# GT-STAR-Lab/MARBLER

Hardware: AMD Instinct MI355X
Metric: env agent-steps/sec (higher is better)
Workload: dtype f32

## Files before the change

marbler_amd/csrc/step_group.h:

```cpp
#pragma once
#include <hip/hip_runtime.h>
#include <stdint.h>

#include <type_traits>

#include "device_common.h"
#include "ipm_qp.h"
#include "lidar.h"
#include "team.h"
#include "probes/diag.h"

namespace rg {

__device__ __forceinline__ void out_store4(float *p, float a, float b, float c, float d) {
    *reinterpret_cast<float4 *>(p) = make_float4(a, b, c, d);
}
__device__ __forceinline__ void out_store1(float *p, float a) {
    *p = a;
}

constexpr int CHUNK = RG_CHUNK;
static_assert(CHUNK >= 1 && CHUNK <= 5, "the sparse collision pre-test covers sub-steps 0..2 and 3..4 of a chunk: longer chunks would go untested");

template <int GW, int QPM = 0, typename QpLds = void, bool SPAN = false>
__device__ __forceinline__ int controller(const rg_scenario_params &p, const Consts &k, int N, int ag, bool lane_ok,
                                          bool upd, float x, float y, float c, float s, float gx, float gy, float &v,
                                          float &w, QpLds *qp RG_CTRL_TICKS_PARAM) {
    RG_CTRL_BEGIN(x, y, c, s)
    const float xix = x + k.pd * c, xiy = y + k.pd * s;
    float ux = gx - xix, uy = gy - xiy;
    {
        const float nrm = norm2_spec(ux, uy);
        const float sc = k.pvl / nrm;
        const bool clip = nrm > k.pvl;
        ux = clip ? ux * sc : ux;
        uy = clip ? uy * sc : uy;
    }
    if constexpr (QPM == RG_QP_CVXOPT) {
        {
            const float n2u = ux * ux + uy * uy;
            const bool clip = n2u > k.bml * k.bml;
            if (__any(clip)) {
                const float sc = k.bml / __builtin_sqrtf(n2u);
                ux = clip ? ux * sc : ux;
                uy = clip ? uy * sc : uy;
            }
        }
        const int lane_ = threadIdx.x;
        qp->rec[lane_] = make_float4(xix, xiy, ux, uy);
        __syncthreads();
        int iters = 0;
        if (upd) iters = ipm::solve_qp_n<GW>(N, ipm::make_consts(p), qp->rec + (lane_ & ~(GW - 1)), qp->ws[lane_ / GW], ag);
        __syncthreads();
        const float4 r = qp->rec[lane_];
        ux = r.z;
        uy = r.w;
        RG_CTRL_TICK(1);
        float vv = c * ux + s * uy;
        float ww = k.inv_pd * (-s * ux + c * uy);
        ww = ww > k.wlim ? k.wlim : ww;
        ww = ww < -k.wlim ? -k.wlim : ww;
        vv = vv > k.vmax ? k.vmax : vv;
        vv = vv < -k.vmax ? -k.vmax : vv;
        ww = ww > k.wmax ? k.wmax : ww;
        ww = ww < -k.wmax ? -k.wmax : ww;
        v = upd ? vv : v;
        w = upd ? ww : w;
        RG_CTRL_TICK(2);
        return iters;
    }
    const float bgain = p.barrier_gain, ugain = p.unsafe_barrier_gain, qp_rtol = p.qp_rtol;
    const int qp_cap = p.qp_max_sweeps;
    const bool has_unsafe = p.barrier_has_unsafe_gain != 0;
    float ex[GW - 1], ey[GW - 1], fx[GW - 1], fy[GW - 1], bp[GW - 1], emax[GW - 1];
    float mu[GW - 1], dmu[GW - 1];
    auto pair_consts = [&](float pxi, float pyi, int K, int i) {
        const float dx = xix - pxi, dy = xiy - pyi;
        const float ee = dx * dx + dy * dy;
        const float h = ee - k.r2;
        const float gain = ((h >= 0.0f) | !has_unsafe) ? bgain : ugain;
        const float b = gain * ((h * h) * h);
        const float n2 = 2.0f * ee;
        const bool ok = lane_ok & ((ag ^ K) < N) & (n2 > 0.0f);
        const float rn2 = ok ? 1.0f / n2 : 0.0f;
        ex[i] = dx;
        ey[i] = dy;
        fx[i] = dx * rn2;
        fy[i] = dy * rn2;
        bp[i] = (0.5f * b) * rn2;
        emax[i] = ok ? fmaxf(__builtin_fabsf(dx), __builtin_fabsf(dy)) : 0.0f;
    };
    const bool helper = SPAN && (threadIdx.x & GW) != 0;
    if constexpr (SPAN) {
        static_assert(GW == 8, "16-lane rows of two 8-lane halves");
        const float mx = mirror_upper_half(xix), my = mirror_upper_half(xiy);
        static_for<0, 4>([&](auto SS) {
            constexpr int S = decltype(SS)::value;
            const int K = helper ? S ^ 7 : S;
            if constexpr (S == 0) pair_consts(mx, my, K, 6);
            else pair_consts(xor_lane<S>(mx), xor_lane<S>(my), K, (S ^ 7) - 1);
        });
        static_for<1, 4>([&](auto SS) {
            constexpr int S = decltype(SS)::value, J = (S ^ 7) - 1;
            ex[S - 1] = ex[J];
            ey[S - 1] = ey[J];
            fx[S - 1] = fx[J];
            fy[S - 1] = fy[J];
            bp[S - 1] = bp[J];
            emax[S - 1] = emax[J];
        });
        static_for<3, 7>([&](auto JJ) {
            constexpr int J = decltype(JJ)::value;
            ex[J] = to_lower_half(ex[J]);
            ey[J] = to_lower_half(ey[J]);
            fx[J] = to_lower_half(fx[J]);
            fy[J] = to_lower_half(fy[J]);
            bp[J] = to_lower_half(bp[J]);
            emax[J] = to_lower_half(emax[J]);
        });
    } else {
        static_for<1, GW>([&](auto KK) {
            constexpr int K = decltype(KK)::value;
            pair_consts(xor_lane<K>(xix), xor_lane<K>(xiy), K, K - 1);
        });
    }
    static_for<0, GW - 1>([&](auto KK) { mu[decltype(KK)::value] = dmu[decltype(KK)::value] = 0.0f; });
    RG_CTRL_PIN_ROUNDS(GW, fx, bp, emax)
    RG_CTRL_TICK(0);
    {
        const float n2u = ux * ux + uy * uy;
        const bool clip = n2u > k.bml * k.bml;
        if (__any(clip)) {
            const float sc = k.bml / __builtin_sqrtf(n2u);
            ux = clip ? ux * sc : ux;
            uy = clip ? uy * sc : uy;
        }
    }
    const float uhx = ux, uhy = uy;
    bool active = upd & !helper;
    int sweeps = 0, my_sweeps = 0;
    auto sweep = [&](auto PH) {
        constexpr int PHASE = decltype(PH)::value;
        ++sweeps;
        if (active) {
            float chg = 0.0f, pa = 0.0f, pb = 0.0f;
            static_for<1, GW>([&](auto KK) {
                constexpr int K = decltype(KK)::value;
                const float pux = xor_lane<K>(ux), puy = xor_lane<K>(uy);
                const float c0 = mu[K - 1] - bp[K - 1];
                const float t = __builtin_fmaf(fy[K - 1], puy - uy, c0);
                float mn = __builtin_fmaf(fx[K - 1], pux - ux, t);
                mn = (mn > 0.0f) ? mn : 0.0f;
                const float delta = mn - mu[K - 1];
                mu[K - 1] = mn;
                ux = __builtin_fmaf(delta, ex[K - 1], ux);
                uy = __builtin_fmaf(delta, ey[K - 1], uy);
                chg = fmaxf(chg, __builtin_fabsf(delta) * emax[K - 1]);
                if constexpr (PHASE == 2) dmu[K - 1] = delta;
                if constexpr (PHASE == 3) {
                    const float dd = delta - dmu[K - 1];
                    pa = __builtin_fmaf(dd, delta, pa);
                    pb = __builtin_fmaf(dd, dd, pb);
                    dmu[K - 1] = delta;
                }
            });
            my_sweeps = sweeps;
            const float um = lane_ok ? fmaxf(__builtin_fabsf(ux), __builtin_fabsf(uy)) : 0.0f;
            const float gchg = group_max_nonneg<GW>(chg);
            const float gum = fmaxf(k.bml, group_max_nonneg<GW>(um));
            active = (gchg > qp_rtol * gum) & (sweeps < qp_cap);
            if constexpr (PHASE == 3) {
                if (active) {
                    const float ga = group_sum<GW>(pa), gb = group_sum<GW>(pb);
                    const bool ok = (gb > 0.0f) & (ga < 0.0f) & (-ga < 32.0f * gb);
                    const float gam = ok ? ga / gb : 0.0f;
                    float sx = uhx, sy = uhy;
                    static_for<1, GW>([&](auto KK) {
                        constexpr int K = decltype(KK)::value;
                        float m = __builtin_fmaf(-gam, dmu[K - 1], mu[K - 1]);
                        m = (m > 0.0f) ? m : 0.0f;
                        mu[K - 1] = m;
                        sx = __builtin_fmaf(m, ex[K - 1], sx);
                        sy = __builtin_fmaf(m, ey[K - 1], sy);
                    });
                    ux = sx;
                    uy = sy;
                }
            }
        }
    };
    if constexpr (SPAN) {
        while (active) {
            sweep(std::integral_constant<int, 1>{});
            if (!active) break;
            sweep(std::integral_constant<int, 2>{});
            if (!active) break;
            sweep(std::integral_constant<int, 3>{});
            if (!active) break;
            sweep(std::integral_constant<int, 0>{});
        }
    } else {
        while (__any(active)) {
            sweep(std::integral_constant<int, 1>{});
            if (!__any(active)) break;
            sweep(std::integral_constant<int, 2>{});
            if (!__any(active)) break;
            sweep(std::integral_constant<int, 3>{});
            if (!__any(active)) break;
            sweep(std::integral_constant<int, 0>{});
        }
    }
    if constexpr (SPAN) {
        ux = to_upper_half(ux);
        uy = to_upper_half(uy);
    }
    RG_CTRL_PIN2(ux, uy);
    RG_CTRL_TICK(1);
    float vv = c * ux + s * uy;
    float ww = k.inv_pd * (-s * ux + c * uy);
    ww = ww > k.wlim ? k.wlim : ww;
    ww = ww < -k.wlim ? -k.wlim : ww;
    vv = vv > k.vmax ? k.vmax : vv;
    vv = vv < -k.vmax ? -k.vmax : vv;
    ww = ww > k.wmax ? k.wmax : ww;
    ww = ww < -k.wmax ? -k.wmax : ww;
    v = upd ? vv : v;
    w = upd ? ww : w;
    RG_CTRL_PIN2(v, w);
    RG_CTRL_COUNT_SWEEPS(sweeps);
    RG_CTRL_TICK(2);
    return my_sweeps;
}

template <int GW, int OD, int NT>
__device__ __forceinline__ void write_neighbour_obs(Lds<GW> &lds, int N, int Knb, int ag, int gbase, bool lane_ok,
                                                    float x, float y, float *obs_row) {
    constexpr int M = NT > 0 ? NT - 1 : GW - 1;
    unsigned long long key[M > 0 ? M : 1];
    bool ok[M > 0 ? M : 1];
    int rank[M > 0 ? M : 1], who[M > 0 ? M : 1];
    static_for<0, M>([&](auto RR) {
        constexpr int r = decltype(RR)::value;
        int j = ag + r + 1;
        j = j >= N ? j - N : j;
        j = j & (GW - 1);
        who[r] = j;
        const float2 pxy = *reinterpret_cast<const float2 *>(&lds.own[gbase + j][0]);
        const float dx = pxy.x - x, dy = pxy.y - y;
        const float d2 = dx * dx + dy * dy;
        ok[r] = lane_ok & (r + 1 < N);
        const unsigned int hi = ok[r] ? __builtin_bit_cast(unsigned int, d2) : 0xFFFFFFFFu;
        key[r] = (static_cast<unsigned long long>(hi) << 32) | static_cast<unsigned int>(j);
        rank[r] = M - 1 - r;
    });
    const bool all_others = Knb >= N - 1;
    static_for<1, M>([&](auto KK) {
        constexpr int k = decltype(KK)::value;
        static_for<0, k>([&](auto QQ) {
            constexpr int q = decltype(QQ)::value;
            const int q_first = key[q] < key[k] ? 1 : 0;
            rank[k] += q_first;
            rank[q] -= q_first;
        });
    });
    float row[M > 0 ? M : 1][OD];
    static_for<0, M>([&](auto RR) {
        constexpr int r = decltype(RR)::value;
        const float *src = &lds.own[gbase + who[r]][0];
        if constexpr (OD == 4) {
            const float4 v = *reinterpret_cast<const float4 *>(src);
            row[r][0] = v.x;
            row[r][1] = v.y;
            row[r][2] = v.z;
            row[r][3] = v.w;
        } else {
#pragma unroll
            for (int c = 0; c < OD; ++c) row[r][c] = src[c];
        }
    });
    static_for<0, M>([&](auto RR) {
        constexpr int r = decltype(RR)::value;
        const int j = who[r];
        const int slot = all_others ? (j < ag ? j : j - 1) : rank[r];
        if (ok[r] & (all_others | (slot < Knb))) {
            float *o = obs_row + (slot + 1) * OD;
            if constexpr (OD == 4) {
                out_store4(o, row[r][0], row[r][1], row[r][2], row[r][3]);
            } else {
#pragma unroll
                for (int c = 0; c < OD; ++c) o[c] = row[r][c];
            }
        }
    });
}

template <int SCN, int GW, bool OBS_ONLY, int NT, bool AHEAD, bool GYM, int QPM = 0, typename QpLds = void, typename Sync = WgSync,
          bool LIDAR = false, bool TEAM = false, bool SPAN = false>
__device__ __forceinline__ void step_once(const KernelArgs &a, Lds<GW> &lds, const StepView &sv, QpLds *qp_lds = nullptr,
                                          const rg_lidar_params *lid = nullptr, const rg_team_params *tm = nullptr) {
    static_assert(!SPAN || (GW == 8 && QPM == 0 && !GYM && !LIDAR && !TEAM), "the 16-lane rows: exact mode, GW = 8, no side blocks");
    constexpr int RW = SPAN ? 2 * GW : GW;
    constexpr int EPW = WAVE / RW;
    RG_STAMPS_BEGIN()
    const rg_scenario_params &p = a.p;
    const Consts &k = a.k;
    const float *q_poses = a.st.poses, *q_carry = a.st.carry_dist, *q_ret = a.st.ep_return, *q_sum = a.st.done_return_sum;
    const int32_t *q_steps = a.st.episode_steps, *q_act = sv.actions, *q_cnt = a.st.done_count, *q_stp = a.st.done_steps_sum;
    int32_t *q_el = GYM ? sv.io.elapsed : nullptr;
    const int q_tl = GYM ? sv.io.time_limit : 0;
    const int32_t *q_rc = a.st.reset_count, *q_nep = AHEAD ? a.st.next_episode : nullptr;
    const float *q_nin = AHEAD ? a.st.next_init : nullptr;
    const int q_nst = AHEAD ? a.next_stride : 0;
    const int q_E = a.E, q_epw = a.envs_per_wave, q_P = p.num_prey, q_N = p.n_agents, q_G = gridDim.x;
    asm volatile("" ::"s"(q_poses), "s"(q_carry), "s"(q_ret), "s"(q_sum), "s"(q_steps), "s"(q_act), "s"(q_cnt), "s"(q_stp),
                 "s"(q_E), "s"(q_epw), "s"(q_P), "s"(q_N), "s"(q_G), "s"(q_rc));
    if constexpr (GYM) asm volatile("" ::"s"(q_el), "s"(q_tl));
    if constexpr (AHEAD) asm volatile("" ::"s"(q_nep), "s"(q_nin), "s"(q_nst));
    const float *q_prey = a.st.prey_loc;
    const uint8_t *q_sen = a.st.prey_sensed, *q_cap = a.st.prey_captured, *q_loaded = a.st.loaded, *q_grid = a.st.grid;
    const uint8_t *q_pix = a.st.pixel_type, *q_reached = a.st.reached_goal;
    const int32_t *q_gcol = a.st.goal_col, *q_msg = a.st.messages, *q_zone = a.st.zone_load, *q_load = a.st.load;
    if constexpr (SCN == RG_SCN_PREDATOR_CAPTURE_PREY) asm volatile("" ::"s"(q_prey), "s"(q_sen), "s"(q_cap));
    else if constexpr (SCN == RG_SCN_WAREHOUSE) asm volatile("" ::"s"(q_loaded));
    else if constexpr (SCN == RG_SCN_SIMPLE) asm volatile("" ::"s"(q_prey));
    else if constexpr (SCN == RG_SCN_ARCTIC_TRANSPORT) asm volatile("" ::"s"(q_grid), "s"(q_pix), "s"(q_reached), "s"(q_gcol));
    else asm volatile("" ::"s"(q_msg), "s"(q_zone), "s"(q_load));
    int32_t *q_tidx = TEAM ? tm->team_index : nullptr;
    const float *q_tstep = TEAM ? tm->agent_step : nullptr, *q_tsr = TEAM ? tm->sensing_radius : nullptr;
    const float *q_tcr = TEAM ? tm->capture_radius : nullptr;
    const int32_t *q_ttq = TEAM ? tm->torque : nullptr;
    const int q_tC = TEAM ? tm->n_sets : 1;
    if constexpr (TEAM) {
        asm volatile("" ::"s"(q_tidx), "s"(q_tstep), "s"(q_tC));
        if constexpr (SCN == RG_SCN_PREDATOR_CAPTURE_PREY) asm volatile("" ::"s"(q_tsr), "s"(q_tcr));
        else if constexpr (SCN == RG_SCN_MATERIAL_TRANSPORT) asm volatile("" ::"s"(q_ttq));
    }

    const int N = NT > 0 ? NT : q_N;
    const int lane = threadIdx.x;
    const int ag = lane & (GW - 1);
    const int g = lane / RW;
    const int gbase = lane & ~(RW - 1);
    const bool helper = SPAN && (lane & GW) != 0;
    const int epw = q_epw > 0 ? q_epw : EPW;
    const int chunk = xcd_chunk(q_G);
    const int e = chunk * epw + g;
    const bool env_ok = (g < epw) & (e < q_E);
    const bool lane_ok = env_ok && ag < N;
    const bool env_st = env_ok & !helper, lane_st = lane_ok & !helper;
    const size_t eN = static_cast<size_t>(e) * N;

#define RG_LATE(v) asm volatile("" : "+v"(v))
    float x = 0.0f, y = 0.0f, th = 0.0f, carry = 0.0f;
    int act = 4;
    int steps_raw = 0;
    float agent_step = 0.0f, sr = 0.0f, cr = 0.0f;
    float st_ret = 0.0f, st_sum = 0.0f;
    int st_cnt = 0, st_steps = 0;
    const bool stats = (!OBS_ONLY) && q_ret != nullptr;
    int pix = 0, reached = 0;
    int team_raw = 0, tq_raw = 0;
    if constexpr (TEAM) {
        if (env_ok) team_raw = q_tidx[e];
    }
    if (lane_ok) {
        const float *X = q_poses + eN * 3;
        x = X[ag];
        y = X[N + ag];
        th = X[2 * N + ag];
        if constexpr (!OBS_ONLY) act = q_act[eN + ag];
        if constexpr (SCN == RG_SCN_ARCTIC_TRANSPORT) pix = q_pix[eN + ag];
        if constexpr (!TEAM) {
        agent_step = p.agent_step[ag];
        if constexpr (SCN == RG_SCN_PREDATOR_CAPTURE_PREY) {
            sr = p.sensing_radius[ag];
            cr = p.capture_radius[ag];
        }
        }
        if constexpr (!OBS_ONLY) carry = q_carry[eN + ag];
        if constexpr (TEAM) {
            const size_t ti = static_cast<size_t>(team_clamp(team_raw, q_tC)) * N + ag;
            agent_step = q_tstep[ti];
            if constexpr (SCN == RG_SCN_PREDATOR_CAPTURE_PREY) {
                sr = q_tsr[ti];
                cr = q_tcr[ti];
            }
            if constexpr (SCN == RG_SCN_MATERIAL_TRANSPORT) tq_raw = q_ttq[ti];
        }
    }
    int rc_raw = -1;
    const bool ahead = AHEAD && (!OBS_ONLY) && q_nst > 0 && a.auto_reset;
    int nx_tag = -2;
    float nx_pose[3] = {0.0f, 0.0f, 0.0f};
    float nx_a = 0.0f, nx_b = 0.0f;
    uint32_t nx_grid[7] = {0, 0, 0, 0, 0, 0, 0};
    auto load_next = [&](bool want) {
        if (want) {
            const float *nb = q_nin + static_cast<size_t>(e) * q_nst;
            if (ag < N) {
                nx_pose[0] = nb[ag];
                nx_pose[1] = nb[N + ag];
                nx_pose[2] = nb[2 * N + ag];
            }
            if constexpr (SCN == RG_SCN_PREDATOR_CAPTURE_PREY || SCN == RG_SCN_SIMPLE) {
                if (ag < q_P) {
                    nx_a = nb[3 * N + 2 * ag];
                    nx_b = nb[3 * N + 2 * ag + 1];
                }
            } else if constexpr (SCN == RG_SCN_MATERIAL_TRANSPORT) {
                if (ag < 2) nx_a = nb[3 * N + ag];
            } else if constexpr (SCN == RG_SCN_ARCTIC_TRANSPORT) {
                const uint32_t *gb = reinterpret_cast<const uint32_t *>(nb + 3 * N);
#pragma unroll
                for (int t = 0; t < 6; ++t) nx_grid[t] = gb[ag * 6 + t];
                nx_grid[6] = gb[24];
            }
        }
    };
    int el_raw = 0;
    if (env_ok) {
        steps_raw = q_steps[e];
        if (!OBS_ONLY && a.auto_reset) rc_raw = q_rc[e];
        if constexpr (GYM) el_raw = q_el[e];
        if (ahead) nx_tag = q_nep[e];
        if (stats && ag == 0) {
            st_ret = q_ret[e];
            st_sum = q_sum[e];
            st_cnt = q_cnt[e];
            st_steps = q_stp[e];
        }
    }
    uint32_t sen_lo = 0, sen_hi = 0, cap_lo = 0, cap_hi = 0;
    int flag_raw[4] = {0, 0, 0, 0};
    int loaded = 0;
    float goal_x = 0.0f, goal_y = 0.0f;
    uint32_t grid_pre[6] = {0, 0, 0, 0, 0, 0};
    int goal_col = 1;
    int load = 0, zone0 = 0, zone1 = 0;
    int msg[4] = {0, 0, 0, 0};
    float2 prey_r[8];
#pragma unroll
    for (int t = 0; t < 8; ++t) prey_r[t] = make_float2(0.0f, 0.0f);
    static_assert(SCN != RG_SCN_ARCTIC_TRANSPORT || GW == 4, "ArcticTransport is a 4-agent scenario");
    if constexpr (SCN == RG_SCN_PREDATOR_CAPTURE_PREY) {
        const int P = q_P;
        if (P <= 8) {
            if (env_ok) {
                const float2 *src = reinterpret_cast<const float2 *>(q_prey) + static_cast<size_t>(e) * P;
#pragma unroll
                for (int t = 0; t < 8; ++t) prey_r[t] = src[t < P ? t : P - 1];
                if (ag < P) {
                    flag_raw[0] = q_sen[static_cast<size_t>(e) * P + ag];
                    flag_raw[1] = q_cap[static_cast<size_t>(e) * P + ag];
                }
                if constexpr (GW < 8)
                    if (ag + GW < P) {
                        flag_raw[2] = q_sen[static_cast<size_t>(e) * P + ag + GW];
                        flag_raw[3] = q_cap[static_cast<size_t>(e) * P + ag + GW];
                    }
            }
        } else {
            if (env_ok) {
                for (int i = ag; i < 2 * P; i += GW) lds.prey[g][i] = q_prey[static_cast<size_t>(e) * 2 * P + i];
                for (int i = ag; i < P; i += GW) {
                    const uint32_t sb = q_sen[static_cast<size_t>(e) * P + i] != 0;
                    const uint32_t cb = q_cap[static_cast<size_t>(e) * P + i] != 0;
                    if (i < 32) {
                        sen_lo |= sb << i;
                        cap_lo |= cb << i;
                    } else {
                        sen_hi |= sb << (i - 32);
                        cap_hi |= cb << (i - 32);
                    }
                }
            }
            sen_lo = group_or<GW>(sen_lo);
            cap_lo = group_or<GW>(cap_lo);
            if (P > 32) {
                sen_hi = group_or<GW>(sen_hi);
                cap_hi = group_or<GW>(cap_hi);
            }
        }
    } else if constexpr (SCN == RG_SCN_WAREHOUSE) {
        if (lane_ok) loaded = q_loaded[eN + ag];
    } else if constexpr (SCN == RG_SCN_SIMPLE) {
        if (env_ok) {
            goal_x = q_prey[static_cast<size_t>(e) * 2];
            goal_y = q_prey[static_cast<size_t>(e) * 2 + 1];
        }
    } else if constexpr (SCN == RG_SCN_ARCTIC_TRANSPORT) {
        if (env_ok) {
            const uint32_t *gsrc = reinterpret_cast<const uint32_t *>(q_grid + static_cast<size_t>(e) * 96);
#pragma unroll
            for (int t = 0; t < 6; ++t) grid_pre[t] = gsrc[ag * 6 + t];
            goal_col = q_gcol[e];
        }
        if (lane_ok) reached = q_reached[eN + ag];
    } else {
        if (env_ok) {
#pragma unroll
            for (int i = 0; i < 4; ++i) {
                if (OBS_ONLY || i >= N) msg[i] = q_msg[4 * e + i];
                else msg[i] = q_act[eN + i];
            }
            zone0 = q_zone[2 * e];
            zone1 = q_zone[2 * e + 1];
        }
        if (lane_ok) load = q_load[eN + ag];
    }

    int viol = 0, max_sweeps = 0;
    bool replayed = false;
    float dist = 0.0f;
    if constexpr (!OBS_ONLY) {
        RG_PIN5(x, y, th, carry, act);
        RG_STAMP(0);
        float gx = x, gy = y;
        {
            const int mv = (SCN == RG_SCN_MATERIAL_TRANSPORT) ? act / 4 : act;
            float sd = agent_step;
            if constexpr (SCN == RG_SCN_ARCTIC_TRANSPORT) {
                const float nrm_s = p.arctic_normal_step, slow_s = p.arctic_slow_step, fast_s = p.arctic_fast_step;
                const float water = pix == 1 ? slow_s : pix == 2 ? fast_s : nrm_s;
                const float ice = pix == 1 ? fast_s : pix == 2 ? slow_s : nrm_s;
                sd = ag < 2 ? fast_s : ag == 3 ? water : ice;
            }
            const float cgx = clamp_spec(gx, p.left, p.right), cgy = clamp_spec(gy, p.up, p.down);
            const float lft = (gx - sd) > p.left ? (gx - sd) : p.left;
            const float rgt = (gx + sd) < p.right ? (gx + sd) : p.right;
            const float upw = (gy - sd) > p.up ? (gy - sd) : p.up;
            const float dwn = (gy + sd) < p.down ? (gy + sd) : p.down;
            gx = mv == 0 ? lft : mv == 1 ? rgt : cgx;
            gy = mv == 2 ? upw : mv == 3 ? dwn : cgy;
        }
        const int thr_pre = __builtin_bit_cast(int, k.thr_pre);
        const int ghost_q = __builtin_bit_cast(int, __builtin_amdgcn_cvt_pkrtz(1000.0f + 32.0f * ag, -1000.0f));
        float v = 0.0f, w = 0.0f, s = 0.0f, c = 1.0f;
        RG_CHUNK_LOCALS()
        RG_CTRL_LOCALS()
        float acc = carry, last = 0.0f;
        bool dead = false;
        float fin_x = 0.0f, fin_y = 0.0f;
        float bx = x, by = y, ox = 0.0f, oy = 0.0f;
        const bool penalize = p.penalize_violations != 0;
        const int U = p.update_frequency, period = p.controller_period;
        for (int it0 = 0; it0 < U; it0 += period) {
            const int n = (U - it0) < period ? (U - it0) : period;
            RG_HEADING_SINCOS(th, s, c);
            const int sw = controller<GW, QPM, QpLds, SPAN>(p, k, N, ag, lane_ok, env_ok & !dead, x, y, c, s, gx, gy, v, w, qp_lds RG_CTRL_TICKS_ARG);
            max_sweeps = sw > max_sweeps ? sw : max_sweeps;
            const float dtv = k.dt * v, dtw = k.dt * w;
            float sd, cd;
            sincos_small_spec(dtw, sd, cd);
            if (__any(__builtin_fabsf(dtw) > 0.25f)) {
                float sd2, cd2;
                sincos_spec(dtw, sd2, cd2);
                const bool big = __builtin_fabsf(dtw) > 0.25f;
                sd = big ? sd2 : sd;
                cd = big ? cd2 : cd;
            }
            if (it0 == 0) RG_STAMP(1);
            const float mrg = __builtin_fmaf((CHUNK - 1) * 1.000001f, __builtin_fabsf(dtv), PRE_SLACK);
            int n_exec = n;
            bool died_now = false;
            const float mstep = lane_ok ? __builtin_fmaf(__builtin_fabsf(k.coll_off), __builtin_fabsf(dtw), __builtin_fabsf(dtv)) * 1.00001f : 0.0f;
            const float M2 = 2.0f * group_max_nonneg<GW>(mstep);
            auto thr_span = [&](int span) {
                const float t = (k.lin_pre + PRE_SLACK) + static_cast<float>(span) * M2;
                return __builtin_bit_cast(int, (t * t) * 1.00002f);
            };
            const int thr_s1 = thr_span(1), thr_s2 = thr_span(2);
            const bool sparse_ok = (k.lin_pre + 2.0f * M2) < 0.24f;

            auto run_chunk = [&](auto CC, int j0) {
                constexpr int C = decltype(CC)::value;
                const float x0 = x, y0 = y, ox0 = ox, oy0 = oy, c0 = c, s0 = s;
                const bool live = lane_ok & !dead;
                int q[C];
                const bool bnd_any = live & ((__builtin_fabsf(x - k.xc) + mrg > k.xh) | (__builtin_fabsf(y - k.yc) + mrg > k.yh));
                static_for<0, C>([&](auto UU) {
                    constexpr int u = decltype(UU)::value;
                    const float fx = __builtin_fmaf(k.coll_off, c, x), fy = __builtin_fmaf(k.coll_off, s, y);
                    const int qr = __builtin_bit_cast(int, __builtin_amdgcn_cvt_pkrtz(fx, fy));
                    q[u] = live ? qr : ghost_q;
                    ox = __builtin_fmaf(c, dtv, ox);
                    oy = __builtin_fmaf(s, dtv, oy);
                    x = bx + ox;
                    y = by + oy;
                    const float cn = __builtin_fmaf(c, cd, -(s * sd));
                    const float sn = __builtin_fmaf(s, cd, c * sd);
                    c = cn;
                    s = sn;
                });
                auto pair_min = [&](int qv) {
                    constexpr bool QUAD_COVER = GW == 8 && NT >= 5 && NT <= 7;
                    constexpr int R = QUAD_COVER ? NT - 1 : GW - 1;
                    int d[R];
                    auto diff = [&](int partner_q) {
                        return __builtin_bit_cast(int, __builtin_bit_cast(half2v, qv) - __builtin_bit_cast(half2v, partner_q));
                    };
                    if constexpr (QUAD_COVER) {
                        static_for<1, 4>([&](auto KK) { d[decltype(KK)::value - 1] = diff(xor_lane_i<decltype(KK)::value>(qv)); });
                        static_for<0, NT - 4>([&](auto MM) { d[3 + decltype(MM)::value] = diff(cross_lane_i<decltype(MM)::value>(qv)); });
                    } else {
                        static_for<1, GW>([&](auto KK) { d[decltype(KK)::value - 1] = diff(xor_lane_i<decltype(KK)::value>(qv)); });
                    }
                    int dm = 0x7FFFFFFF;
                    dot2_batch<R>(d);
#pragma unroll
                    for (int r = 0; r < R; ++r) dm = d[r] < dm ? d[r] : dm;
                    return dm;
                };
                int dmin_u[C];
                bool sparse_hit = live & !sparse_ok;
                {
                    constexpr int SPAN0 = C - 1 < 2 ? C - 1 : 2;
                    const int t0 = SPAN0 == 0 ? thr_pre : SPAN0 == 1 ? thr_s1 : thr_s2;
                    if constexpr (SPAN && C >= 4) {
                        const int t3 = C == 4 ? thr_pre : thr_s1;
                        const int dm = pair_min(helper ? q[3] : q[0]);
                        sparse_hit = sparse_hit | (dm <= (helper ? t3 : t0));
                        dmin_u[0] = dmin_u[3] = dm;
                    } else {
                        dmin_u[0] = pair_min(q[0]);
                        sparse_hit = sparse_hit | (dmin_u[0] <= t0);
                        if constexpr (C >= 4) {
                            const int t3 = C == 4 ? thr_pre : thr_s1;
                            dmin_u[3] = pair_min(q[3]);
                            sparse_hit = sparse_hit | (dmin_u[3] <= t3);
                        }
                    }
                }
                if (penalize && __any(sparse_hit | bnd_any)) {
                RG_CHUNK_DENSE_BEGIN()
                if constexpr (SPAN && C >= 4) {
                    const int mine = dmin_u[0], other = xor_lane_i<8>(mine);
                    dmin_u[0] = helper ? other : mine;
                    dmin_u[3] = helper ? mine : other;
                }
                if constexpr (SPAN && C >= 3) {
                    const int mine = pair_min(helper ? q[2] : q[1]), other = xor_lane_i<8>(mine);
                    if constexpr (C == 5) dmin_u[4] = pair_min(q[4]);
                    dmin_u[1] = helper ? other : mine;
                    dmin_u[2] = helper ? mine : other;
                } else {
                    static_for<1, C>([&](auto UU) {
                        constexpr int u = decltype(UU)::value;
                        if constexpr (u != 3) dmin_u[u] = pair_min(q[u]);
                    });
                }
                int dmin = dmin_u[0];
                static_for<1, C>([&](auto UU) { dmin = dmin_u[decltype(UU)::value] < dmin ? dmin_u[decltype(UU)::value] : dmin; });
                RG_CHUNK_DENSE_END(dmin)
                if (__any((dmin <= thr_pre) | bnd_any)) {
                    replayed = true;
                    float rx = x0, ry = y0, rox = ox0, roy = oy0, rc = c0, rs = s0;
                    static_for<0, C>([&](auto UU) {
                        constexpr int u = decltype(UU)::value;
                        const bool bnd = lane_ok & !dead & ((rx < k.xmin) | (rx > k.xmax) | (ry < k.ymin) | (ry > k.ymax));
                        const float fx = __builtin_fmaf(k.coll_off, rc, rx), fy = __builtin_fmaf(k.coll_off, rs, ry);
                        bool col = false;
                        if (!__any(dmin_u[u] <= thr_pre)) {
                        } else if constexpr (GW == 8 && NT >= 5 && NT <= 7) {
                            static_for<1, 4>([&](auto KK) {
                                constexpr int K = decltype(KK)::value;
                                const float dx = fx - xor_lane<K>(fx), dy = fy - xor_lane<K>(fy);
                                col = col | (((ag ^ K) < N) & (dx * dx + dy * dy <= k.coll_lim2));
                            });
                            static_for<0, NT - 4>([&](auto MM) {
                                constexpr int M = decltype(MM)::value;
                                const float dx = fx - cross_lane<M>(fx), dy = fy - cross_lane<M>(fy);
                                col = col | (dx * dx + dy * dy <= k.coll_lim2);
                            });
                        } else {
                            static_for<1, GW>([&](auto KK) {
                                constexpr int K = decltype(KK)::value;
                                const float dx = fx - xor_lane<K>(fx), dy = fy - xor_lane<K>(fy);
                                col = col | (((ag ^ K) < N) & (dx * dx + dy * dy <= k.coll_lim2));
                            });
                        }
                        col = col & lane_ok & !dead;
                        const int code = (group_any<GW>(col, gbase) ? 1 : 0) | (group_any<GW>(bnd, gbase) ? 2 : 0);
                        rox = __builtin_fmaf(rc, dtv, rox);
                        roy = __builtin_fmaf(rs, dtv, roy);
                        rx = bx + rox;
                        ry = by + roy;
                        if (env_ok & !dead & (code != 0)) {
                            viol = code;
                            n_exec = j0 + u + 1;
                            died_now = true;
                            dead = true;
                            fin_x = rx;
                            fin_y = ry;
                        }
                        const float cn = __builtin_fmaf(rc, cd, -(rs * sd));
                        const float sn = __builtin_fmaf(rs, cd, rc * sd);
                        rc = cn;
                        rs = sn;
                    });
                    RG_CHUNK_REPLAY_END(rx, ry)
                }
                }
            };
            int j = 0;
            for (; j + CHUNK <= n; j += CHUNK) run_chunk(std::integral_constant<int, CHUNK>{}, j);
            static_for<1, CHUNK>([&](auto RR) {
                if (n - j == decltype(RR)::value) run_chunk(RR, j);
            });

            const bool upd = env_ok & (!dead | died_now);
            const float ne = static_cast<float>(n_exec);
            const float adv = __builtin_fabsf(dtv);
            th = upd ? wrap_spec(__builtin_fmaf(ne, dtw, th)) : th;
            acc = upd ? __builtin_fmaf(ne, adv, acc) : acc;
            last = upd ? adv : last;
            {
                const float tx = x - bx, ty = y - by;
                ox = (bx - (x - tx)) + (ox - tx);
                oy = (by - (y - ty)) + (oy - ty);
                bx = x;
                by = y;
            }
            if (it0 == 0) RG_STAMP(2);
            if (!__any(env_ok & !dead)) break;
        }
        if (dead) {
            x = fin_x;
            y = fin_y;
        }
        dist = viol ? acc : acc - last;
        carry = last;
        RG_STAMP(3);
        RG_CTRL_REPORT()
        RG_CHUNK_REPORT()
    }

    const int D = p.obs_dim;
    float *obs_row = sv.io.obs + (eN + ag) * D;
    bool done = false;
    int remaining = -1;
    float reward = 0.0f;
    RG_LATE(steps_raw);
    const int steps = steps_raw + (OBS_ONLY ? 0 : 1);
    RG_LATE(rc_raw);
    RG_LATE(nx_tag);
    const bool have_next = ahead & (nx_tag == rc_raw);
    const bool next_early = env_ok & have_next & ((viol != 0) | (steps > p.max_episode_steps));
    if constexpr (AHEAD) load_next(next_early & !helper);

    if constexpr (SCN == RG_SCN_PREDATOR_CAPTURE_PREY) {
        const int P = q_P;
        if constexpr (TEAM) {
            RG_LATE(sr);
            RG_LATE(cr);
        }
        const float sr2 = sr * sr, cr2 = cr * cr;
        if (P > 8) Sync::sync();
        if (P <= 8) {
            RG_LATE(flag_raw[0]);
            RG_LATE(flag_raw[1]);
            uint32_t sb = (flag_raw[0] != 0 ? 1u : 0u) << ag, cb = (flag_raw[1] != 0 ? 1u : 0u) << ag;
            if constexpr (GW < 8) {
                RG_LATE(flag_raw[2]);
                RG_LATE(flag_raw[3]);
                sb |= (flag_raw[2] != 0 ? 1u : 0u) << (ag + GW);
                cb |= (flag_raw[3] != 0 ? 1u : 0u) << (ag + GW);
            }
            sen_lo = group_or<GW>(sb);
            cap_lo = group_or<GW>(cb);
        }
        uint32_t nsen_lo = sen_lo, nsen_hi = sen_hi, ncap_lo = cap_lo, ncap_hi = cap_hi;
        auto scan = [&](int lo, int hi, auto &&f) {
            for (int i0 = lo; i0 < hi; i0 += 4) {
                float2 pl[4];
#pragma unroll
                for (int t = 0; t < 4; ++t) {
                    const int i = (i0 + t) < hi ? (i0 + t) : (hi - 1);
                    pl[t] = *reinterpret_cast<const float2 *>(&lds.prey[g][2 * i]);
                }
#pragma unroll
                for (int t = 0; t < 4; ++t) {
                    const float dx = x - pl[t].x, dy = y - pl[t].y;
                    f(i0 + t, (i0 + t) < hi, pl[t].x, pl[t].y, dx * dx + dy * dy);
                }
            }
        };
        float closest = -1.0f, qx = -5.0f, qy = -5.0f;
        if (P <= 8) {
            const float2 (&pl)[8] = prey_r;
            float d2[8];
            uint32_t s_b = 0, c_b = 0;
            const bool acts = lane_ok & (act == 4);
#pragma unroll
            for (int t = 0; t < 8; ++t) {
                const float dx = x - pl[t].x, dy = y - pl[t].y;
                d2[t] = dx * dx + dy * dy;
                const bool in = t < P;
                s_b |= ((in & lane_ok & (d2[t] <= sr2)) ? 1u : 0u) << t;
                c_b |= ((in & acts & (d2[t] <= cr2)) ? 1u : 0u) << t;
            }
            if constexpr (!OBS_ONLY) {
                s_b = group_or<GW>(s_b);
                c_b = group_or<GW>(c_b);
                nsen_lo = sen_lo | (s_b & ~cap_lo);
                ncap_lo = cap_lo | (nsen_lo & c_b & ~cap_lo);
                if (env_st && ag < P) {
                    a.st.prey_sensed[static_cast<size_t>(e) * P + ag] = (nsen_lo >> ag) & 1u;
                    a.st.prey_captured[static_cast<size_t>(e) * P + ag] = (ncap_lo >> ag) & 1u;
                }
                if constexpr (GW < 8)
                    if (env_ok && ag + GW < P) {
                        a.st.prey_sensed[static_cast<size_t>(e) * P + ag + GW] = (nsen_lo >> (ag + GW)) & 1u;
                        a.st.prey_captured[static_cast<size_t>(e) * P + ag + GW] = (ncap_lo >> (ag + GW)) & 1u;
                    }
            }
#pragma unroll
            for (int t = 0; t < 8; ++t) {
                const bool cap = ((ncap_lo >> t) & 1u) != 0;
                const bool take = (t < P) & !cap & (d2[t] <= sr2) & ((d2[t] < closest) | (closest == -1.0f));
                qx = take ? pl[t].x : qx;
                qy = take ? pl[t].y : qy;
                closest = take ? d2[t] : closest;
            }
        } else {
        if constexpr (!OBS_ONLY) {
            uint32_t s_lo = 0, s_hi = 0, c_lo = 0, c_hi = 0;
            const bool acts = lane_ok & (act == 4);
            const int P32 = P < 32 ? P : 32;
            scan(0, P32, [&](int i, bool in, float, float, float d2) {
                s_lo |= ((in & lane_ok & (d2 <= sr2)) ? 1u : 0u) << (i & 31);
                c_lo |= ((in & acts & (d2 <= cr2)) ? 1u : 0u) << (i & 31);
            });
            s_lo = group_or<GW>(s_lo);
            c_lo = group_or<GW>(c_lo);
            nsen_lo = sen_lo | (s_lo & ~cap_lo);
            ncap_lo = cap_lo | (nsen_lo & c_lo & ~cap_lo);
            if (P > 32) {
                scan(32, P, [&](int i, bool in, float, float, float d2) {
                    s_hi |= ((in & lane_ok & (d2 <= sr2)) ? 1u : 0u) << ((i - 32) & 31);
                    c_hi |= ((in & acts & (d2 <= cr2)) ? 1u : 0u) << ((i - 32) & 31);
                });
                s_hi = group_or<GW>(s_hi);
                c_hi = group_or<GW>(c_hi);
                nsen_hi = sen_hi | (s_hi & ~cap_hi);
                ncap_hi = cap_hi | (nsen_hi & c_hi & ~cap_hi);
            }
            if (env_st) {
                for (int i = ag; i < P; i += GW) {
                    const uint32_t sw_ = i < 32 ? nsen_lo >> i : nsen_hi >> (i - 32);
                    const uint32_t cw_ = i < 32 ? ncap_lo >> i : ncap_hi >> (i - 32);
                    a.st.prey_sensed[static_cast<size_t>(e) * P + i] = sw_ & 1u;
                    a.st.prey_captured[static_cast<size_t>(e) * P + i] = cw_ & 1u;
                }
            }
        }
        {
            auto nearest = [&](uint32_t capmask, int base) {
                return [&, capmask, base](int i, bool in, float px, float py, float d2) {
                    const bool cap = ((capmask >> ((i - base) & 31)) & 1u) != 0;
                    const bool take = in & !cap & (d2 <= sr2) & ((d2 < closest) | (closest == -1.0f));
                    qx = take ? px : qx;
                    qy = take ? py : qy;
                    closest = take ? d2 : closest;
                };
            };
            scan(0, P < 32 ? P : 32, nearest(ncap_lo, 0));
            if (P > 32) scan(32, P, nearest(ncap_hi, 32));
        }
        }
        RG_STAMP_E(0);
        const int od = p.capability_aware ? 6 : 4;
        lds.own[lane][0] = x;
        lds.own[lane][1] = y;
        lds.own[lane][2] = qx;
        lds.own[lane][3] = qy;
        lds.own[lane][4] = sr;
        lds.own[lane][5] = cr;
        Sync::sync();
        if (od == 6) {
            if (lane_st) {
#pragma unroll
                for (int cc = 0; cc < 6; ++cc) obs_row[cc] = lds.own[lane][cc];
            }
            write_neighbour_obs<GW, 6, NT>(lds, N, p.num_neighbors, ag, gbase, lane_st, x, y, obs_row);
        } else {
            if (lane_st) out_store4(obs_row, x, y, qx, qy);
            write_neighbour_obs<GW, 4, NT>(lds, N, p.num_neighbors, ag, gbase, lane_st, x, y, obs_row);
        }
        RG_STAMP_E(1);
        if constexpr (!OBS_ONLY) {
            const int unseen0 = P - __builtin_popcount(sen_lo) - __builtin_popcount(sen_hi);
            const int left0 = P - __builtin_popcount(cap_lo) - __builtin_popcount(cap_hi);
            const int unseen1 = P - __builtin_popcount(nsen_lo) - __builtin_popcount(nsen_hi);
            const int left1 = P - __builtin_popcount(ncap_lo) - __builtin_popcount(ncap_hi);
            if (viol) {
                reward = p.violation_reward;
                done = true;
            } else {
                reward = 0.0f;
                reward = reward + static_cast<float>(unseen0 - unseen1) * p.sense_reward;
                reward = reward + static_cast<float>(left0 - left1) * p.capture_reward;
                reward = reward + p.time_penalty;
                if (steps > p.max_episode_steps || left1 == 0) {
                    done = true;
                    remaining = left1;
                }
            }
        }
    } else if constexpr (SCN == RG_SCN_WAREHOUSE) {
        lds.own[lane][0] = x;
        lds.own[lane][1] = y;
        lds.own[lane][2] = loaded ? 1.0f : 0.0f;
        Sync::sync();
        if (lane_st) {
            obs_row[0] = x;
            obs_row[1] = y;
            obs_row[2] = loaded ? 1.0f : 0.0f;
        }
        write_neighbour_obs<GW, 3, NT>(lds, N, p.num_neighbors, ag, gbase, lane_st, x, y, obs_row);
        if constexpr (!OBS_ONLY) {
            if (viol) {
                reward = p.violation_reward;
                done = true;
            } else {
                const bool green = (ag % 2) == 0;
                if (loaded) {
                    if (x < -1.5f + p.goal_width && ((green && y > 0.0f) || (!green && y <= 0.0f))) {
                        reward = p.unload_reward;
                        loaded = 0;
                    }
                } else {
                    if (x > 1.5f - p.goal_width && ((!green && y > 0.0f) || (green && y <= 0.0f))) {
                        reward = p.load_reward;
                        loaded = 1;
                    }
                }
                done = steps > p.max_episode_steps;
                if (lane_st) a.st.loaded[eN + ag] = static_cast<uint8_t>(loaded);
            }
        }
    } else if constexpr (SCN == RG_SCN_SIMPLE) {
        lds.own[lane][0] = x;
        lds.own[lane][1] = y;
        Sync::sync();
        if (lane_st) {
            obs_row[0] = x;
            obs_row[1] = y;
            obs_row[2 * N] = goal_x;
            obs_row[2 * N + 1] = goal_y;
        }
        write_neighbour_obs<GW, 2, NT>(lds, N, N - 1, ag, gbase, lane_st, x, y, obs_row);
        if constexpr (!OBS_ONLY) {
            if (viol) {
                reward = p.violation_reward;
                done = true;
            } else {
                const float dx = x - goal_x, dy = y - goal_y;
                const float r = -(dx * dx + dy * dy);
                reward = r * p.reward_scaler;
                done = steps > p.max_episode_steps;
            }
        }
    } else if constexpr (SCN == RG_SCN_ARCTIC_TRANSPORT) {
        {
            uint32_t *gdst = reinterpret_cast<uint32_t *>(&lds.grid[g][0]);
#pragma unroll
            for (int t = 0; t < 6; ++t) gdst[ag * 6 + t] = grid_pre[t];
        }
        Sync::sync();
        const uint8_t *grid = &lds.grid[g][0];
        int row = -static_cast<int>((y - 1.0f) / 0.25f), col = static_cast<int>((x + 1.5f) / 0.25f);
        row = row < 0 ? 0 : row > 7 ? 7 : row;
        col = col < 0 ? 0 : col > 11 ? 11 : col;
        if constexpr (!OBS_ONLY) {
            pix = grid[row * 12 + col];
            reached = reached | (pix == 3 ? 1 : 0);
        }
        const int here = grid[row * 12 + col];
        lds.own[lane][0] = x;
        lds.own[lane][1] = y;
        lds.own[lane][2] = static_cast<float>(here);
        lds.aload[lane] = row * 16 + col;
        Sync::sync();
        const float goalx = static_cast<float>(goal_col) * 0.25f - 1.5f, goaly = -1.0f * 0.25f + 0.75f;
        if (lane_ok) {
            obs_row[0] = x;
            obs_row[1] = y;
            obs_row[2] = static_cast<float>(here);
            const int o0 = ag == 0 ? 1 : ag == 1 ? 0 : ag == 2 ? 3 : 2;
            const int o1 = ag < 2 ? 2 : 0, o2 = ag < 2 ? 3 : 1;
            const int oth[3] = {o0, o1, o2};
#pragma unroll
            for (int m = 0; m < 3; ++m) {
                obs_row[3 + 3 * m + 0] = lds.own[gbase + oth[m]][0];
                obs_row[3 + 3 * m + 1] = lds.own[gbase + oth[m]][1];
                obs_row[3 + 3 * m + 2] = lds.own[gbase + oth[m]][2];
            }
            obs_row[12] = goalx;
            obs_row[13] = goaly;
#pragma unroll
            for (int i = 0; i < 2; ++i) {
                const int rc = lds.aload[gbase + i];
                const int r_ = rc >> 4, c_ = rc & 15;
                const int left = c_ > 0 ? c_ - 1 : c_, right = c_ < 11 ? c_ + 1 : c_;
                const int up = r_ > 0 ? r_ - 1 : r_, down = r_ < 7 ? r_ + 1 : r_;
                float *o = obs_row + 14 + 8 * i;
                o[0] = static_cast<float>(grid[up * 12 + left]);
                o[1] = static_cast<float>(grid[r_ * 12 + left]);
                o[2] = static_cast<float>(grid[down * 12 + left]);
                o[3] = static_cast<float>(grid[up * 12 + c_]);
                o[4] = static_cast<float>(grid[down * 12 + c_]);
                o[5] = static_cast<float>(grid[up * 12 + right]);
                o[6] = static_cast<float>(grid[r_ * 12 + right]);
                o[7] = static_cast<float>(grid[down * 12 + right]);
            }
        }
        if constexpr (LIDAR) write_lidar<SCN, GW, OBS_ONLY, Sync>(*lid, a, lds, lane, gbase, N, ag, lane_ok, x, y, th, obs_row);
        if constexpr (!OBS_ONLY) {
            const float dx = x - goalx, dy = y - goaly;
            lds.ax[lane] = dx * dx + dy * dy;
            lds.ay[lane] = static_cast<float>(pix * 2 + reached);
            Sync::sync();
            if (viol) {
                reward = p.violation_reward;
                done = true;
            } else {
                reward = 0.0f;
                bool all_reached = true;
#pragma unroll
                for (int j = 2; j < 4; ++j) {
                    const int pr = static_cast<int>(lds.ay[gbase + j]);
                    const bool rj = (pr & 1) != 0;
                    if (!rj) reward = reward + p.not_reached_penalty;
                    if ((pr >> 1) != 3) reward = reward + p.dist_multiplier * lds.ax[gbase + j];
                    all_reached = all_reached && rj;
                }
                done = steps > p.max_episode_steps;
                if (!done) done = all_reached;
            }
            if (lane_ok) {
                a.st.pixel_type[eN + ag] = static_cast<uint8_t>(pix);
                a.st.reached_goal[eN + ag] = static_cast<uint8_t>(reached);
            }
        }
    } else {
#pragma unroll
        for (int i = 0; i < 4; ++i) {
            RG_LATE(msg[i]);
            if (!OBS_ONLY && i < N) msg[i] = msg[i] % 4;
        }
        if constexpr (TEAM) RG_LATE(tq_raw);
        if (lane_st) {
            obs_row[0] = x;
            obs_row[1] = y;
            obs_row[2] = static_cast<float>(load);
            obs_row[3] = static_cast<float>(zone0);
            obs_row[4] = static_cast<float>(zone1);
#pragma unroll
            for (int i = 0; i < 4; ++i) obs_row[5 + i] = static_cast<float>(msg[i]);
            if (p.capability_aware) {
                if constexpr (TEAM) obs_row[9] = static_cast<float>(tq_raw);
                else obs_row[9] = static_cast<float>(p.torque[ag]);
                obs_row[10] = agent_step;
            }
        }
        if constexpr (!OBS_ONLY) {
            lds.ax[lane] = x;
            lds.ay[lane] = y;
            lds.aload[lane] = load;
            if constexpr (TEAM) team_lds<SCN, GW>().torque[lane] = tq_raw;
            Sync::sync();
            if (viol) {
                reward = p.violation_reward;
                done = true;
            } else {
                reward = p.time_penalty;
                const float egw = p.end_goal_width;
                const float zr2 = p.zone1_radius * p.zone1_radius;
                bool any_load = false;
                for (int j = 0; j < N; ++j) {
                    const float jx = lds.ax[gbase + j], jy = lds.ay[gbase + j];
                    int jl = lds.aload[gbase + j];
                    int tq;
                    if constexpr (TEAM) tq = team_lds<SCN, GW>().torque[gbase + j];
                    else tq = p.torque[j];
                    if (jl > 0) {
                        if (jx < -1.5f + egw) {
                            reward = reward + static_cast<float>(jl) * p.unload_multiplier;
                            jl = 0;
                        }
                    } else {
                        if (jx > 1.5f - egw) {
                            if (zone1 > tq) {
                                jl = tq;
                                zone1 -= tq;
                            } else {
                                jl = zone1;
                                zone1 = 0;
                            }
                            reward = reward + static_cast<float>(jl) * p.load_multiplier;
                        } else if (jx * jx + jy * jy <= zr2) {
                            if (zone0 > tq) {
                                jl = tq;
                                zone0 -= tq;
                            } else {
                                jl = zone0;
                                zone0 = 0;
                            }
                            reward = reward + static_cast<float>(jl) * p.load_multiplier;
                        }
                    }
                    if (j == ag) load = jl;
                    any_load = any_load || (jl != 0);
                }
                done = steps > p.max_episode_steps;
                if (!done) done = (zone0 == 0 && zone1 == 0 && !any_load);
            }
            int total = 0;
            {
                lds.aload[lane] = lane_ok ? load : 0;
                Sync::sync();
                for (int j = 0; j < N; ++j) total += lds.aload[gbase + j];
            }
            if (done) remaining = zone0 + zone1 + total;
            if (lane_st) a.st.load[eN + ag] = load;
            if (lane_st && ag == 0) {
                a.st.zone_load[2 * e] = zone0;
                a.st.zone_load[2 * e + 1] = zone1;
            }
            if (lane_st && ag < 4) a.st.messages[4 * e + ag] = msg[ag == 0 ? 0 : ag == 1 ? 1 : ag == 2 ? 2 : 3];
        }
    }

    if constexpr (LIDAR && SCN != RG_SCN_ARCTIC_TRANSPORT) write_lidar<SCN, GW, OBS_ONLY, Sync>(*lid, a, lds, lane, gbase, N, ag, lane_ok, x, y, th, obs_row);
    RG_STAMP(4);
    if constexpr (!OBS_ONLY) {
        constexpr bool gym = GYM;
        bool trunc = false;
        if (gym) {
            RG_LATE(el_raw);
            trunc = env_ok & !done & (el_raw + 1 >= q_tl);
        }
        const bool ended = done | trunc;
        float rsum = 0.0f;
        if ((stats && !p.shared_reward) || gym) {
            Sync::sync();
            lds.ax[lane] = lane_ok ? reward : 0.0f;
            Sync::sync();
            for (int j = 0; j < N; ++j) rsum = rsum + lds.ax[gbase + j];
        }
        if (lane_st) {
            float *X = a.st.poses + eN * 3;
            X[ag] = x;
            X[N + ag] = y;
            X[2 * N + ag] = th;
            a.st.carry_dist[eN + ag] = carry;
            out_store1(sv.io.reward + eN + ag, reward);
            out_store1(sv.io.dist_travelled + eN + ag, dist);
            if (ag == 0) {
                a.st.episode_steps[e] = steps;
                if (stats) {
                    RG_LATE(st_ret);
                    RG_LATE(st_sum);
                    RG_LATE(st_cnt);
                    RG_LATE(st_steps);
                    float ret = st_ret + (p.shared_reward ? reward : rsum);
                    if (ended) {
                        a.st.done_return_sum[e] = st_sum + ret;
                        a.st.done_count[e] = st_cnt + 1;
                        a.st.done_steps_sum[e] = st_steps + steps;
                        ret = 0.0f;
                    }
                    a.st.ep_return[e] = ret;
                }
                sv.io.done[e] = done ? 1 : 0;
                if (gym) {
                    q_el[e] = ended ? 0 : el_raw + 1;
                    sv.io.truncated[e] = trunc ? 1 : 0;
                    sv.io.ended[e] = ended ? 1 : 0;
                    sv.io.reward_sum[e] = rsum;
                }
                sv.io.violation[e] = static_cast<uint8_t>(viol);
                sv.io.remaining[e] = remaining;
                if (sv.io.qp_sweeps) sv.io.qp_sweeps[e] = max_sweeps;
            }
            if constexpr (GYM) {
                if (sv.io.zero_obs_on_end && ended) {
                    for (int c = 0; c < D; ++c) obs_row[c] = 0.0f;
                }
            }
        }
        RG_STAMP(5);
        if (a.auto_reset && __any(env_ok & ended)) {
            Sync::sync();
            if constexpr (AHEAD) load_next(env_st & ended & have_next & !next_early);
            if (__any(env_ok & ended & !have_next)) reset_group<SCN, GW, Sync>(a, lds, e, g, ag, env_st & ended & !have_next, rc_raw);
            if (env_st & ended & have_next) {
                if (ag < N) {
                    float *X = a.st.poses + eN * 3;
                    X[ag] = nx_pose[0];
                    X[N + ag] = nx_pose[1];
                    X[2 * N + ag] = nx_pose[2];
                    a.st.carry_dist[eN + ag] = 0.0f;
                    if constexpr (SCN == RG_SCN_WAREHOUSE) a.st.loaded[eN + ag] = 0;
                    if constexpr (SCN == RG_SCN_MATERIAL_TRANSPORT) {
                        a.st.load[eN + ag] = 0;
                        if (ag < 4) a.st.messages[4 * e + ag] = 0;
                    }
                    if constexpr (SCN == RG_SCN_ARCTIC_TRANSPORT) {
                        a.st.pixel_type[eN + ag] = 0;
                        a.st.reached_goal[eN + ag] = 0;
                    }
                }
                if constexpr (SCN == RG_SCN_PREDATOR_CAPTURE_PREY || SCN == RG_SCN_SIMPLE) {
                    const int P = q_P;
                    const float *nb = q_nin + static_cast<size_t>(e) * q_nst + 3 * N;
                    for (int i = ag; i < P; i += GW) {
                        float *pl = a.st.prey_loc + (static_cast<size_t>(e) * P + i) * 2;
                        pl[0] = i == ag ? nx_a : nb[2 * i];
                        pl[1] = i == ag ? nx_b : nb[2 * i + 1];
                        if constexpr (SCN == RG_SCN_PREDATOR_CAPTURE_PREY) {
                            a.st.prey_sensed[static_cast<size_t>(e) * P + i] = 0;
                            a.st.prey_captured[static_cast<size_t>(e) * P + i] = 0;
                        }
                    }
                } else if constexpr (SCN == RG_SCN_MATERIAL_TRANSPORT) {
                    if (ag < 2) a.st.zone_load[2 * e + ag] = __builtin_bit_cast(int32_t, nx_a);
                } else if constexpr (SCN == RG_SCN_ARCTIC_TRANSPORT) {
                    uint32_t *gd = reinterpret_cast<uint32_t *>(a.st.grid + static_cast<size_t>(e) * 96);
#pragma unroll
                    for (int t = 0; t < 6; ++t) gd[ag * 6 + t] = nx_grid[t];
                    if (ag == 0) a.st.goal_col[e] = static_cast<int32_t>(nx_grid[6]);
                }
                if (ag == 0) {
                    a.st.reset_count[e] = rc_raw + 1;
                    a.st.episode_steps[e] = 0;
                }
            }
            if constexpr (TEAM) {
                if (env_ok & ended & (ag == 0)) q_tidx[e] = team_draw(*tm, static_cast<uint64_t>(a.env_offset + e), rc_raw, a.seed);
            }
        }
        if (AHEAD && ahead && !(replayed | __any(max_sweeps > 2)) && __any(env_ok & !ended & !have_next)) {
            const bool need = env_st & !ended & !have_next;
            Sync::sync();
            reset_group<SCN, GW, Sync>(a, lds, e, g, ag, need, rc_raw, reset_dst_next(a, e));
            if (need && ag == 0) a.st.next_episode[e] = rc_raw;
        }
        RG_STAMP(6);
        RG_STAMPS_WRITE(lane, sv.io.qp_sweeps, chunk * EPW, a.E, max_sweeps)
    }
}

struct PlainFamily {
// ... 186 lines not shown
```

Baseline: 1.703 billion.

## Split neighbour-obs ranking and prey sensing across SPAN helper lanes

In SPAN mode, each agent's neighbour-ranking work is split between the primary lane and its helper lane (lane ^ GW). Each lane handles half the candidates and uses cross-lane exchanges to complete the ranks. Prey sensing and capture for P<=8 is also split, with each lane checking four prey and merging the masks and closest-prey results through xor-lane shuffles. This reduces per-lane unrolled work and register pressure, at the cost of extra cross-lane shuffles and only helps when SPAN is enabled.

New measurement: 1.793 billion (median of 6 runs). 1.05x the previous value.

```diff
diff --git a/marbler_amd/csrc/step_group.h b/marbler_amd/csrc/step_group.h
--- a/marbler_amd/csrc/step_group.h
+++ b/marbler_amd/csrc/step_group.h
@@ -232,29 +232,37 @@
     return my_sweeps;
 }
 
-template <int GW, int OD, int NT>
+template <int GW, int OD, int NT, bool SPAN = false>
 __device__ __forceinline__ void write_neighbour_obs(Lds<GW> &lds, int N, int Knb, int ag, int gbase, bool lane_ok,
                                                     float x, float y, float *obs_row) {
     constexpr int M = NT > 0 ? NT - 1 : GW - 1;
-    unsigned long long key[M > 0 ? M : 1];
-    bool ok[M > 0 ? M : 1];
-    int rank[M > 0 ? M : 1], who[M > 0 ? M : 1];
-    static_for<0, M>([&](auto RR) {
-        constexpr int r = decltype(RR)::value;
+    constexpr int S = SPAN ? (M + 1) / 2 : M;
+    const int r0 = SPAN && (threadIdx.x & GW) != 0 ? S : 0;
+    unsigned long long key[S > 0 ? S : 1], okey[S > 0 ? S : 1];
+    bool ok[S > 0 ? S : 1];
+    int rank[S > 0 ? S : 1], who[S > 0 ? S : 1];
+    static_for<0, S>([&](auto RR) {
+        constexpr int l = decltype(RR)::value;
+        const int r = r0 + l;
         int j = ag + r + 1;
         j = j >= N ? j - N : j;
         j = j & (GW - 1);
-        who[r] = j;
+        who[l] = j;
         const float2 pxy = *reinterpret_cast<const float2 *>(&lds.own[gbase + j][0]);
         const float dx = pxy.x - x, dy = pxy.y - y;
         const float d2 = dx * dx + dy * dy;
-        ok[r] = lane_ok & (r + 1 < N);
-        const unsigned int hi = ok[r] ? __builtin_bit_cast(unsigned int, d2) : 0xFFFFFFFFu;
-        key[r] = (static_cast<unsigned long long>(hi) << 32) | static_cast<unsigned int>(j);
-        rank[r] = M - 1 - r;
+        ok[l] = lane_ok & (r + 1 < N);
+        if constexpr (SPAN) ok[l] &= r < M;
+        const unsigned int hi = ok[l] ? __builtin_bit_cast(unsigned int, d2) : 0xFFFFFFFFu;
+        key[l] = (static_cast<unsigned long long>(hi) << 32) | static_cast<unsigned int>(j);
+        if constexpr (SPAN) {
+            const unsigned int ohi = static_cast<unsigned int>(xor_lane_i<8>(static_cast<int>(hi)));
+            okey[l] = (static_cast<unsigned long long>(ohi) << 32) | static_cast<unsigned int>(xor_lane_i<8>(j));
+        }
+        rank[l] = S - 1 - l;
     });
     const bool all_others = Knb >= N - 1;
-    static_for<1, M>([&](auto KK) {
+    static_for<1, S>([&](auto KK) {
         constexpr int k = decltype(KK)::value;
         static_for<0, k>([&](auto QQ) {
             constexpr int q = decltype(QQ)::value;
@@ -263,8 +271,14 @@
             rank[q] -= q_first;
         });
     });
-    float row[M > 0 ? M : 1][OD];
-    static_for<0, M>([&](auto RR) {
+    if constexpr (SPAN) {
+        static_for<0, S>([&](auto LL) {
+            constexpr int l = decltype(LL)::value;
+            static_for<0, S>([&](auto QQ) { rank[l] += okey[decltype(QQ)::value] < key[l] ? 1 : 0; });
+        });
+    }
+    float row[S > 0 ? S : 1][OD];
+    static_for<0, S>([&](auto RR) {
         constexpr int r = decltype(RR)::value;
         const float *src = &lds.own[gbase + who[r]][0];
         if constexpr (OD == 4) {
@@ -278,7 +292,7 @@
             for (int c = 0; c < OD; ++c) row[r][c] = src[c];
         }
     });
-    static_for<0, M>([&](auto RR) {
+    static_for<0, S>([&](auto RR) {
         constexpr int r = decltype(RR)::value;
         const int j = who[r];
         const int slot = all_others ? (j < ag ? j : j - 1) : rank[r];
@@ -348,6 +362,7 @@
     const bool env_ok = (g < epw) & (e < q_E);
     const bool lane_ok = env_ok && ag < N;
     const bool env_st = env_ok & !helper, lane_st = lane_ok & !helper;
+    const bool lane_nb = SPAN ? lane_ok : lane_st;
     const size_t eN = static_cast<size_t>(e) * N;
 
 #define RG_LATE(v) asm volatile("" : "+v"(v))
@@ -447,8 +462,14 @@
         if (P <= 8) {
             if (env_ok) {
                 const float2 *src = reinterpret_cast<const float2 *>(q_prey) + static_cast<size_t>(e) * P;
+                if constexpr (SPAN) {
+                    const int t0 = helper ? 4 : 0;
+#pragma unroll
+                    for (int t = 0; t < 4; ++t) prey_r[t] = src[t0 + t < P ? t0 + t : P - 1];
+                } else {
 #pragma unroll
                 for (int t = 0; t < 8; ++t) prey_r[t] = src[t < P ? t : P - 1];
+                }
                 if (ag < P) {
                     flag_raw[0] = q_sen[static_cast<size_t>(e) * P + ag];
                     flag_raw[1] = q_cap[static_cast<size_t>(e) * P + ag];
@@ -786,7 +807,47 @@
             }
         };
         float closest = -1.0f, qx = -5.0f, qy = -5.0f;
-        if (P <= 8) {
+        if (SPAN && P <= 8) {
+            const float2 (&pl)[8] = prey_r;
+            const int t0 = helper ? 4 : 0;
+            const bool acts = lane_ok & (act == 4);
+            const float sr2e = lane_ok ? sr2 : -1.0f, cr2e = acts ? cr2 : -1.0f;
+            float d2[4];
+            uint32_t m = 0;
+#pragma unroll
+            for (int t = 0; t < 4; ++t) {
+                const float dx = x - pl[t].x, dy = y - pl[t].y;
+                d2[t] = dx * dx + dy * dy;
+                m |= (d2[t] <= sr2e ? 1u : 0u) << t;
+                m |= (d2[t] <= cr2e ? 1u : 0u) << (8 + t);
+            }
+            m <<= t0;
+            m = group_or<GW>(m);
+            m |= static_cast<uint32_t>(xor_lane_i<8>(static_cast<int>(m)));
+            const uint32_t in_p = (1u << P) - 1u;
+            if constexpr (!OBS_ONLY) {
+                const uint32_t s_b = m & in_p, c_b = (m >> 8) & in_p;
+                nsen_lo = sen_lo | (s_b & ~cap_lo);
+                ncap_lo = cap_lo | (nsen_lo & c_b & ~cap_lo);
+                if (env_st && ag < P) {
+                    a.st.prey_sensed[static_cast<size_t>(e) * P + ag] = (nsen_lo >> ag) & 1u;
+                    a.st.prey_captured[static_cast<size_t>(e) * P + ag] = (ncap_lo >> ag) & 1u;
+                }
+            }
+            const uint32_t cap_l = (ncap_lo | ~in_p) >> t0;
+#pragma unroll
+            for (int t = 0; t < 4; ++t) {
+                const bool cap = ((cap_l >> t) & 1u) != 0;
+                const bool take = !cap & (d2[t] <= sr2) & ((d2[t] < closest) | (closest == -1.0f));
+                qx = take ? pl[t].x : qx;
+                qy = take ? pl[t].y : qy;
+                closest = take ? d2[t] : closest;
+            }
+            const float o_closest = xor_lane<8>(closest), o_qx = xor_lane<8>(qx), o_qy = xor_lane<8>(qy);
+            const bool other = (o_closest != -1.0f) & ((closest == -1.0f) | (o_closest < closest));
+            qx = other ? o_qx : qx;
+            qy = other ? o_qy : qy;
+        } else if (P <= 8) {
             const float2 (&pl)[8] = prey_r;
             float d2[8];
             uint32_t s_b = 0, c_b = 0;
@@ -882,10 +943,10 @@
 #pragma unroll
                 for (int cc = 0; cc < 6; ++cc) obs_row[cc] = lds.own[lane][cc];
             }
-            write_neighbour_obs<GW, 6, NT>(lds, N, p.num_neighbors, ag, gbase, lane_st, x, y, obs_row);
+            write_neighbour_obs<GW, 6, NT, SPAN>(lds, N, p.num_neighbors, ag, gbase, lane_nb, x, y, obs_row);
         } else {
             if (lane_st) out_store4(obs_row, x, y, qx, qy);
-            write_neighbour_obs<GW, 4, NT>(lds, N, p.num_neighbors, ag, gbase, lane_st, x, y, obs_row);
+            write_neighbour_obs<GW, 4, NT, SPAN>(lds, N, p.num_neighbors, ag, gbase, lane_nb, x, y, obs_row);
         }
         RG_STAMP_E(1);
         if constexpr (!OBS_ONLY) {
@@ -917,7 +978,7 @@
             obs_row[1] = y;
             obs_row[2] = loaded ? 1.0f : 0.0f;
         }
-        write_neighbour_obs<GW, 3, NT>(lds, N, p.num_neighbors, ag, gbase, lane_st, x, y, obs_row);
+        write_neighbour_obs<GW, 3, NT, SPAN>(lds, N, p.num_neighbors, ag, gbase, lane_nb, x, y, obs_row);
         if constexpr (!OBS_ONLY) {
             if (viol) {
                 reward = p.violation_reward;
@@ -949,7 +1010,7 @@
             obs_row[2 * N] = goal_x;
             obs_row[2 * N + 1] = goal_y;
         }
-        write_neighbour_obs<GW, 2, NT>(lds, N, N - 1, ag, gbase, lane_st, x, y, obs_row);
+        write_neighbour_obs<GW, 2, NT, SPAN>(lds, N, N - 1, ag, gbase, lane_nb, x, y, obs_row);
         if constexpr (!OBS_ONLY) {
             if (viol) {
                 reward = p.violation_reward;
```
